# nash169/manifold-gp

Measured on AMD Instinct MI355X. Metric: CG-solve wall-time + SpMV HBM GB/s, N=60k RMNIST graph, higher is better.
Workload: dtype f32; 1 GPU; C3 RMNIST-like N=60000 d=784 k=50 nu=2 randomwalk; nodes=60000, edges=1777442, nnz_padded=3667592, rhs_columns=1, system=A = I + noise*outputscale*Q, Q=(2nu/kappa^2 I + L)^nu x D, solver=CG on A (Chronopoulos-Gear, one hipGraph per solve)

## Files before the change

include/mgp_hip.h:

```cpp
#ifndef MGP_HIP_H
#define MGP_HIP_H

#include <stddef.h>
#include <stdint.h>

#ifdef __cplusplus
extern "C" {
#endif

#define MGP_OK 0
#define MGP_ERR_ARG (-1)
#define MGP_ERR_WORKSPACE (-2)
#define MGP_ERR_UNSUPPORTED (-3)
#define MGP_ERR_NOT_CONVERGED (-4)
#define MGP_ERR_KNN_AMBIGUOUS (-5)
#define MGP_ERR_TIMEOUT (-6)

#define MGP_PAD 4

int mgp_version(void);
int mgp_device_info(int* cu_count, int* wave_size, size_t* hbm_bytes);

size_t mgp_knn_workspace_bytes(int64_t N, int64_t n, int d, int k);
int mgp_knn_search(const float* db, int64_t N, int d, const float* q, int64_t n, int k,
// ... 53 lines not shown
typedef struct {
  int64_t n;
  const int32_t* rowptr;
  const int32_t* col;
  const float* vals;
  const float* diag;
  int64_t ncols;
  const int32_t* tile_ptr;
  const int32_t* tile_cols;
  const uint16_t* lid;
  int32_t tile_rows;
  int32_t tile_max_cols;
  int32_t tile_max_entries;
  int32_t spmv_lanes;
  const int32_t* tile_rowptr;
  const float* tile_vals;
  const int32_t* tile_rowid;
  const int32_t* mt_sptr;
  const int32_t* mt_dcol;
  const float* mt_img;
  int32_t mt_tiles;
  int32_t mt_steps;
} mgp_csr_t;

int mgp_spmm_dot_blocks_csr(const mgp_csr_t* L, int C);
int mgp_spmm_set_tile_mode(int on);
int mgp_spmm_set_tile_loop_mode(int on);
int mgp_spmm_set_tile_small_mode(int on);
int mgp_spmm_set_tile_wide_mode(int on);
int mgp_spmm_set_dict_mode(int on);
int mgp_spmm_set_mt_mode(int on);
int mgp_spmm_kernel_choice(const mgp_csr_t* L, int C, int with_dot, int64_t row_offset);
int mgp_spmm_mt_fill(int64_t n, const int32_t* rowptr, const float* vals, const uint16_t* lid16, const int32_t* tile_ptr16,
                     const int32_t* tile_cols16, const int32_t* sptr, int64_t steps, int32_t* dcol, float* img, void* stream);
int mgp_spmm_timing_begin(int max_launches);
int mgp_spmm_timing_end(float* total_ms, int* launches);
int mgp_spmm_set_v4_mode(int on);

int mgp_spmm_dot_blocks(int64_t n, int C);
int mgp_spmm_set_group_hint(int lanes);
int mgp_spmm_set_rows_in_flight(int rows);
int mgp_spmm_fused(const mgp_csr_t* L, const float* X, int C, float* Y, float a, float b,
                   const float* pre, const float* post, const float* base, float cb, float co,
                   const float* dotw, float* dot_partials, void* stream);

int mgp_spmm_fused_rows(const mgp_csr_t* L_local, int64_t row_offset, const float* X, int C, float* Y,
// ... 239 lines not shown
```

manifold_gp_amd/_lib.py:

```python
import ctypes
import os
import threading
from ctypes import (POINTER, Structure, byref, c_double, c_float, c_int, c_int32, c_int64, c_size_t,
                    c_uint64, c_void_p)

import torch

_HERE = os.path.dirname(os.path.abspath(__file__))
LIB_PATH = os.path.join(_HERE, "libmgp_hip.so")
_LIB = None
_LOCK = threading.Lock()

MGP_ERRORS = {
    -1: "MGP_ERR_ARG (null pointer / bad size / bad enum)",
    -2: "MGP_ERR_WORKSPACE (work buffer too small)",
    -3: "MGP_ERR_UNSUPPORTED",
    -4: "MGP_ERR_NOT_CONVERGED",
    -5: "MGP_ERR_KNN_AMBIGUOUS",
}


class MgpError(RuntimeError):
    def __init__(self, fn, code):
        self.code = code
        what = MGP_ERRORS.get(code, "hipError_t %d" % code if code > 0 else "error %d" % code)
        super().__init__("%s failed: %s" % (fn, what))


class CsrT(Structure):
    _fields_ = [("n", c_int64), ("rowptr", c_void_p), ("col", c_void_p), ("vals", c_void_p),
                ("diag", c_void_p),
                ("ncols", c_int64), ("tile_ptr", c_void_p), ("tile_cols", c_void_p), ("lid", c_void_p),
                ("tile_rows", c_int32), ("tile_max_cols", c_int32), ("tile_max_entries", c_int32),
                ("spmv_lanes", c_int32), ("tile_rowptr", c_void_p), ("tile_vals", c_void_p),
                ("tile_rowid", c_void_p),
                ("mt_sptr", c_void_p), ("mt_dcol", c_void_p), ("mt_img", c_void_p), ("mt_tiles", c_int32), ("mt_steps", c_int32)]


class OperatorT(Structure):
    _fields_ = [("L", CsrT), ("pre", c_void_p), ("post", c_void_p), ("nu", c_int32),
                ("kappa", c_float), ("scale", c_float), ("form", c_int32), ("noise", c_float),
                ("obs_w", c_void_p)]


class CgParamsT(Structure):
    _fields_ = [("tol", c_float), ("max_iter", c_int32), ("min_iter", c_int32),
                ("stop_mode", c_int32), ("check_every", c_int32), ("use_graph", c_int32),
                ("max_refine", c_int32)]


class LanczosParamsT(Structure):
    _fields_ = [("max_basis", c_int32), ("degree", c_int32), ("max_restarts", c_int32),
                ("tol", c_float), ("seed", c_uint64)]


_P = c_void_p
SIGNATURES = {
    "mgp_version": (c_int, []),
    "mgp_device_info": (c_int, [POINTER(c_int), POINTER(c_int), POINTER(c_size_t)]),
# ... 261 lines not shown


def release_workspace(tag, device=None):
    for key in [k for k in _WORK if k[0] == tag and (device is None or k[1] == str(device))]:
        del _WORK[key]


_LEAKED = []


def leak(*objects):
    _LEAKED.extend(objects)


def csr_struct(n, rowptr, col, vals, diag, ncols=0, tiles=None, tile_vals=None, mt=None, lanes=0):
    s = CsrT(int(n), rowptr.data_ptr(), col.data_ptr(), vals.data_ptr(), diag.data_ptr(), int(ncols))
    s.spmv_lanes = int(lanes)
    if tiles is not None and (tiles.get("rowid") is None or tile_vals is not None):
        s.tile_ptr, s.tile_cols, s.lid = tiles["tile_ptr"].data_ptr(), tiles["tile_cols"].data_ptr(), tiles["lid"].data_ptr()
        s.tile_rows, s.tile_max_cols, s.tile_max_entries = tiles["rows"], tiles["max_cols"], tiles["max_entries"]
        if tiles.get("rowid") is not None:
            s.tile_rowptr, s.tile_rowid = tiles["tile_rowptr"].data_ptr(), tiles["rowid"].data_ptr()
            s.tile_vals = tile_vals.data_ptr()
    if mt is not None:
        s.mt_sptr, s.mt_dcol, s.mt_img = mt.sptr.data_ptr(), mt.dcol.data_ptr(), mt.img.data_ptr()
        s.mt_tiles, s.mt_steps = mt.tiles, mt.steps
    return s
```

manifold_gp_amd/csrc/cg.hip:

```cpp
#include <math.h>
#include <chrono>
#include <mutex>
#include <new>
#include <vector>
#include <string.h>
#include <algorithm>
#include "mgp_common.h"
#include "mgp_internal.h"
#include "cg_rule.h"
#include "cg_policy.h"
#include "cg_handoff.h"

namespace {

#ifndef MGP_LAB_UPD
#define MGP_LAB_UPD 0
#endif

typedef float mgp_cg_v4f __attribute__((ext_vector_type(4)));

struct CgArgs {
  int64_t n;
  int C, TC, TS;
  float *x, *r, *u, *w, *p, *s;
// ... 1334 lines not shown

extern "C" int mgp_cg_plan_create(const mgp_operator_t* op, int C, const float* minv,
                                  const mgp_cg_params_t* params, void* work, size_t work_bytes,
                                  void* stream, void** plan_out) {
  return plan_create_impl(op, C, minv, params, nullptr, work, work_bytes, stream, plan_out);
}

extern "C" int mgp_cg_plan_rebind(void* plan, const mgp_operator_t* op, const float* minv) {
  CgPlan* pl = static_cast<CgPlan*>(plan);
  if (!pl || !op) return MGP_ERR_ARG;
  if (pl->poisoned || pl->is_dist) return MGP_ERR_UNSUPPORTED;
  const mgp_operator_t& o = pl->op;
  const bool same = op->L.n == o.L.n && op->L.ncols == o.L.ncols && op->nu == o.nu && op->form == o.form &&
                    (op->form != 3 || ((op->obs_w != nullptr) == (o.obs_w != nullptr))) &&
                    (op->pre != nullptr) == (o.pre != nullptr) && (op->post != nullptr) == (o.post != nullptr) &&
                    (minv != nullptr) == (pl->args.minv != nullptr) &&
                    (op->L.tile_ptr != nullptr) == (o.L.tile_ptr != nullptr) && op->L.tile_rows == o.L.tile_rows &&
                    op->L.tile_max_cols == o.L.tile_max_cols && op->L.tile_max_entries == o.L.tile_max_entries &&
                    (op->L.tile_rowptr != nullptr) == (o.L.tile_rowptr != nullptr) &&
                    (op->L.tile_vals != nullptr) == (o.L.tile_vals != nullptr) &&
                    (op->L.tile_rowid != nullptr) == (o.L.tile_rowid != nullptr) &&
                    (op->L.mt_img != nullptr) == (o.L.mt_img != nullptr) && op->L.mt_tiles == o.L.mt_tiles &&
                    op->L.mt_steps == o.L.mt_steps && op->L.spmv_lanes == o.L.spmv_lanes &&
                    mgp_spmm_dot_blocks_for(&op->L, pl->C) == pl->nb_loc &&
                    (!pl->ch.fold || op->pre == op->post);
  if (!same) return MGP_ERR_UNSUPPORTED;
  if (pl->ch.cx) {
    const float cc = op->noise * op->scale;
    if (!(cc > 0.f)) return MGP_ERR_UNSUPPORTED;
    pl->opB = cx_operator(op);
    if (mgp_spmm_dot_blocks_for(&pl->opB.L, 4) != pl->cxa.nbs4) return MGP_ERR_UNSUPPORTED;
    pl->cxa.sigma = sqrtf(cc);
  }
  pl->op = mgp_operator_copy(op);
  pl->args.minv = minv;
  pl->args.pre = op->pre;
  pl->rebound = true;
  return MGP_OK;
}

extern "C" size_t mgp_cg_dist_workspace_bytes(const mgp_operator_t* op_local, int C, int world) {
  if (!op_local || C <= 0 || C > kMaxC || op_local->L.n <= 0 || world < 1 || !mgp_spmv_lanes_ok(op_local->L.spmv_lanes)) return 0;
  return cg_bytes(op_local, C, world, true);
}

extern "C" int mgp_cg_plan_create_dist(const mgp_operator_t* op_local, int C, const float* minv,
// ... 240 lines not shown
```

manifold_gp_amd/csrc/spmm.hip:

```cpp
#include <string.h>
#include <atomic>
#include <type_traits>
#include "mgp_common.h"
#include "mgp_internal.h"
#include "cg_rule.h"
#include "cg_handoff.h"
#include <hip/hip_ext.h>
#include <vector>

namespace {

constexpr int kBlock = 256;
constexpr int kMaxGrid = 4096;

struct SpmmArgs {
  int64_t n;
  const int32_t* rowptr;
  const int32_t* col;
  const float* vals;
  const float* diag;
  const float* X;
  float* Y;
  int C;
  float a, b;
// ... 189 lines not shown
  int zero;
  const unsigned grid_x = gridDim.x;
#define MGP_TILE_HEAD_ARGS                                                                                                     \
  "s"(p.n), "s"(p.rowptr), "s"(t.rowptr_t), "s"(p.vals), "s"(t.vals_t), "s"(p.diag), "s"(p.X), "s"(p.post), "s"(p.a), "s"(p.b),   \
      "s"(p.cb), "s"(p.co), "s"(t.tile_ptr), "s"(t.tile_cols), "s"(t.lid), "s"(t.max_cols), "s"(t.rowid), "s"(grid_x),           \
      "s"(PRE ? p.pre : nullptr), "s"(CBV ? p.cbv : nullptr), "s"(ONE ? (int64_t)0 : t.ntiles), "s"(ONE ? 0 : t.tiles_per_block)
  if constexpr (!STEP) {
    asm("s_mov_b32 %0, 0" : "=s"(zero) : MGP_TILE_HEAD_ARGS, "s"(p.goff), "s"(p.base), "s"(p.dotw), "s"(p.Y), "s"(p.dot_partials),
        "s"(p.copy_x), "s"(p.dot2_partials), "s"(p.skip), "s"(p.tick), "s"(p.tick_reset));
  } else {
    asm("s_mov_b32 %0, 0" : "=s"(zero) : MGP_TILE_HEAD_ARGS, "s"(cs.r), "s"(cs.x), "s"(cs.p), "s"(cs.s), "s"(cs.us), "s"(cs.pre),
        "s"(cs.pd_rr), "s"(cs.pd_delta), "s"(cs.nbs), "s"(cs.blk), "s"(cs.state), "s"(cs.host_state), "s"(cs.host_resid),
        "s"(cs.arrive), "s"(cs.tol), "s"(cs.max_iter), "s"(cs.min_iter), "s"(cs.stop_mode), "s"(cs.dcoef), "s"(cs.dgamma));
  }
#undef MGP_TILE_HEAD_ARGS
  const int32_t* __restrict__ rowptr = t.rowptr_t ? t.rowptr_t : p.rowptr;
  const float* __restrict__ vals = t.vals_t ? t.vals_t : p.vals;
  const int lane0 = __builtin_amdgcn_mbcnt_lo(0u, 0u) + zero;
  const int* __restrict__ skip_ptr = (p.skip ? p.skip : reinterpret_cast<const int*>(rowptr)) + lane0;
  const int* __restrict__ tick_ptr = (p.tick ? p.tick : reinterpret_cast<const int*>(rowptr)) + lane0;
  int skipl = 0, tickl = 0;
  constexpr int TR = BS / 4;
  constexpr int NQ = 4;
  const int lb = mgp_xcd_block(blockIdx.x, grid_x) + zero;
  const int tid = threadIdx.x, sub = tid & 3;
#ifdef MGP_STAMP
  int* st_base = !pa.stamp_on ? nullptr : (p.skip ? const_cast<int*>(p.skip) - 1 : p.tick);
  if (st_base && blockIdx.x == 0 && tid == 0) {
    const int si = atomicAdd(st_base + 8, 1);
    reinterpret_cast<unsigned long long*>(st_base + 16)[si & 255] = wall_clock64() * 8 + 0;
  }
  if (st_base && tid == 0 && blockIdx.x < 2048) reinterpret_cast<unsigned long long*>(st_base + 16)[256 + 2 * blockIdx.x] = wall_clock64();
#endif
  float* __restrict__ xl = tile_lds;
  float* __restrict__ part = tile_lds + t.max_cols;
  const float* __restrict__ x = p.X;
  const float* __restrict__ prev = p.pre;
  const int32_t* __restrict__ tile_ptr = t.tile_ptr;
  const uint32_t* __restrict__ tile_cols = reinterpret_cast<const uint32_t*>(t.tile_cols);
  const uint16_t* __restrict__ lid = t.lid;
  float dsum = 0.f, dsum2 = 0.f;
  const int64_t t0 = ONE ? (int64_t)lb : (int64_t)lb * t.tiles_per_block;
  const int64_t t1 = ONE ? t0 + 1 : (t0 + t.tiles_per_block < t.ntiles ? t0 + t.tiles_per_block : t.ntiles);
  __shared__ float cg_sh_w[MODE == kTileCgStep ? BS / MGP_WAVE : 1][3];
  __shared__ float cg_sh_o[MODE == kTileCgStep ? BS / MGP_WAVE : 1];
  __shared__ int cg_sh_state[MODE == kTileCgStep ? 2 : 1];
// ... 25 lines not shown
  };
  [[maybe_unused]] float cg_go0 = 0.f, cg_go1 = 0.f, cg_ao0 = 0.f, cg_ao1 = 0.f, cg_bb_old = 0.f;
  [[maybe_unused]] int cg_st_it = 0, cg_st_done = 0;
  [[maybe_unused]] mgp_v8i cg_blk;
  [[maybe_unused]] auto take_blk = [&]() {
    asm("" : "+s"(cg_blk));
    const CgScalars sc = __builtin_bit_cast(CgScalars, cg_blk);
    cg_go0 = sc.go0; cg_go1 = sc.go1; cg_ao0 = sc.ao0; cg_ao1 = sc.ao1; cg_bb_old = sc.bb; cg_st_it = sc.it; cg_st_done = sc.done;
  };
  [[maybe_unused]] float cg_alpha = 0.f, cg_beta = 0.f, cg_bb = 0.f, cg_nrr = 0.f;
  [[maybe_unused]] int cg_it = 0;
  [[maybe_unused]] bool cg_fresh = false;
  if constexpr (MODE == kTileCgStep) {
    static_assert(BS == 256, "the step's sums are written for four waves");
    static_assert(sizeof(CgScalars) == sizeof(mgp_v8i) && alignof(CgScalars) == alignof(mgp_v8i), "the scalar block is one load");
    cg_blk = *reinterpret_cast<const mgp_v8i*>(cs.blk);
    if constexpr (!ONE) take_blk();
    if constexpr (!CG_LATE) { cg_request_partials(); cg_sum_partials(); }
  }
  [[maybe_unused]] auto zero_x = [&]() {
    if constexpr (STEP) {
      for (int64_t tl = t0; tl < t1; ++tl) {
        const int64_t pos = tl * TR + tid;
        if (tid < TR && pos < p.n) cs.x[t.rowid ? (int64_t)t.rowid[pos] : pos] = 0.f;
      }
    }
  };
  for (int64_t tile = t0; tile < t1; ++tile) {
    if constexpr (!STEP) {
      skipl = *skip_ptr;
      tickl = *tick_ptr;
    }
    const int64_t r0 = tile * TR;
    const int64_t r1 = r0 + TR < p.n ? r0 + TR : p.n;
    const int e0 = rowptr[r0], e1 = rowptr[r1];
    const int dp = tile_ptr[tile];
    const int D = tile_ptr[tile + 1] - dp;
    const int qb = e0 >> 2, Q = (e1 - e0) >> 2;
    __builtin_amdgcn_sched_barrier(0);
    if constexpr (STEP && ONE) take_blk();
    unsigned c[NQ];
#pragma unroll
    for (int k = 0; k < NQ; ++k) {
      const int j = tid + k * BS;
      c[k] = (unsigned)tile_cols[j < D ? dp + j : 0];
    }
    __builtin_amdgcn_sched_barrier(0);
    mgp_v4f v[NQ];
    mgp_v4h l[NQ];
#pragma unroll
    for (int k = 0; k < NQ / 2; ++k) {
      const int q = tid + k * BS;
      const int qi = q < Q ? qb + q : 0;
      v[k] = *reinterpret_cast<const mgp_v4f*>(vals + 4 * (int64_t)qi);
      l[k] = *reinterpret_cast<const mgp_v4h*>(lid + 4 * (int64_t)qi);
    }
    __builtin_amdgcn_sched_barrier(0);
    float g[NQ];
#pragma unroll
    for (int k = 0; k < NQ; ++k) {
      g[k] = x[c[k]];
      if (PRE) g[k] *= prev[c[k]];
    }
    __builtin_amdgcn_sched_barrier(0);
#pragma unroll
    for (int k = NQ / 2; k < NQ; ++k) {
      const int q = tid + k * BS;
      const int qi = q < Q ? qb + q : 0;
      v[k] = *reinterpret_cast<const mgp_v4f*>(vals + 4 * (int64_t)qi);
      l[k] = *reinterpret_cast<const mgp_v4h*>(lid + 4 * (int64_t)qi);
    }
    __builtin_amdgcn_sched_barrier(0);
    const int64_t row = r0 + (tid >> 2);
    const bool valid = row < r1;
    const int64_t pr = valid ? row : r0;
    const int64_t rr = t.rowid ? (int64_t)t.rowid[pr] : pr;
    const int64_t grr = rr + p.goff;
    const int rs = rowptr[pr], re = rowptr[pr + 1];
    const float raw_x = x[grr];
    float e_x = raw_x;
    if (PRE) e_x *= prev[grr];
    const float e_diag = p.diag[rr];
    const float l_post = (p.post ? p.post : x)[grr], l_base = (p.base ? p.base : x)[grr], l_dotw = (p.dotw ? p.dotw : x)[grr];
    const float e_post = p.post ? l_post : 1.f;
    const float e_base = p.base ? l_base : 0.f;
    const float e_dotw = p.dotw ? l_dotw : 0.f;
    const float e_cb = CBV ? p.cbv[grr] : p.cb;
    [[maybe_unused]] float f_r = 0.f, f_s = 0.f, f_p = 0.f, f_x = 0.f, f_pre = 1.f;
    if constexpr (MODE == kTileCgStep) {
      f_r = cs.r[grr]; f_s = cs.s[grr]; f_p = cs.p[grr]; f_x = cs.x[grr];
      const float l_pre = (cs.us ? cs.pre : x)[grr];
      f_pre = cs.us ? l_pre : 1.f;
    }
    __builtin_amdgcn_sched_barrier(0);
    if (p.skip && skipl) return;
    if constexpr (MODE == kTileCgStep) {
      if (tile == t0) {
        if constexpr (CG_LATE) cg_request_partials();
        __builtin_amdgcn_sched_barrier(0);
// ... 1144 lines not shown
    return MGP_ERR_ARG;
  hipStream_t st = mgp_stream(stream);
  MGP_HIP_TRY(hipMemsetAsync(img, 0, (size_t)(steps + 32) * 256, st));
  MGP_HIP_TRY(hipMemsetAsync(dcol + 4 * steps, 0, 192 * sizeof(int32_t), st));
  hipLaunchKernelGGL(spmm_mt_fill_kernel, dim3((unsigned)mgp_cdiv(n + 15, kBlock)), dim3(kBlock), 0, st, n, rowptr, vals, lid16,
                     tile_ptr16, tile_cols16, sptr, dcol, img);
  MGP_LAUNCH_CHECK();
  return MGP_OK;
}


static int spmm_cols_group(int C) {
  int g = 4;
  while (g < C && g < 64) g <<= 1;
  return g;
}

static int spmm_rows_per_pass(int C, int lanes, int rows_in_flight) {
  if (C == 1) return (kBlock / lanes) * rows_in_flight;
  if (C <= 16 && (C & 3) == 0) return (kBlock / 16) * 4;
  return kBlock / spmm_cols_group(C) * 4;
}

static size_t tile_lds_bytes(const mgp_csr_t* L) {
  return ((size_t)L->tile_max_cols + (size_t)(L->tile_max_entries >> 2)) * sizeof(float);
}

static int tile_grid(const mgp_csr_t* L, int* tiles_per_block) {
  const int64_t ntiles = mgp_cdiv(L->n, L->tile_rows);
  const int64_t tpb = mgp_cdiv(ntiles, kMaxGrid);
  if (tiles_per_block) *tiles_per_block = (int)tpb;
  return (int)mgp_cdiv(ntiles, tpb);
}

static int tile_small_window(const mgp_csr_t* L) {
  const int max_q = L->tile_max_entries >> 2;
  const long budget = 40448 - (long)L->tile_max_cols * 16;
  long w = budget > 0 ? budget / 16 / 256 * 256 : 0;
  if (w < 1024) w = 1024;
  if (w > max_q) w = (max_q + 255) / 256 * 256;
  return (int)(w > 0 ? w : 256);
}
static size_t tile_small_lds_bytes(const mgp_csr_t* L, int C) {
  const size_t max_q = (size_t)(L->tile_max_entries >> 2), w = (size_t)tile_small_window(L);
  size_t b = ((size_t)L->tile_max_cols + (max_q < w ? max_q : w)) * 16;
  const size_t red = (size_t)64 * C * sizeof(float);
  return b > red ? b : red;
}

static int tile_wide_cap(const mgp_csr_t* L) {
  int cap = (L->tile_max_cols + 63) / 64 * 64;
// ... 19 lines not shown
  if (s > need) s = need;
  return (int)s;
}
static size_t dict_lds_bytes(const mgp_csr_t* L, int C) {
  const size_t d = (size_t)(dict_slots(L, C) + 1) * dict_nv(C) * 256 + (size_t)dict_stream_cap(L) * 6;
  const size_t red = (size_t)64 * dict_nv(C) * 256;
  return d > red ? d : red;
}
static int dict_grid(const mgp_csr_t* L) {
  const int64_t ntiles = mgp_cdiv(L->n, L->tile_rows);
  return (int)(ntiles < kMaxGrid ? ntiles : kMaxGrid);
}

constexpr int kMtMinCols = 48;
static bool mt_image_fits(const mgp_csr_t* L, int C) {
  if (!L->mt_img || !L->mt_sptr || !L->mt_dcol || L->mt_tiles <= 0 || L->mt_steps <= 0) return false;
  if (C < kMtMinCols || C > 256 || (C & 3) != 0 || L->tile_rowid) return false;
  if (L->ncols != 0 && L->ncols != L->n) return false;
  if ((int64_t)L->n * C * 4 >= (int64_t(1) << 31) || ((int64_t)L->mt_steps + 32) * 256 >= (int64_t(1) << 31)) return false;
  if ((L->mt_steps & 15) != 0) return false;
  return L->mt_tiles == (int32_t)mgp_cdiv(L->n, 16);
}

static TileArgs tile_args(const mgp_csr_t* L, int tiles_per_block, int part_window) {
  return TileArgs{L->tile_ptr, L->tile_cols, L->lid, mgp_cdiv(L->n, L->tile_rows), tiles_per_block, L->tile_max_cols,
                  L->tile_rowptr, L->tile_vals, L->tile_rowid, L->tile_max_entries, part_window};
}

namespace {
enum class SpmmFamily { RowGroups, Gather, TileC1, TileSmall, MatrixCore, Dict, TileWide };

struct SpmmPlan {
  int err;
  SpmmFamily family;
  int grid;
  size_t lds;
  int dot_blocks;
  bool align16;
  int64_t rows_per_block;
  int lanes, rows_in_flight;
  bool v4_ok;
  int tiles_per_block;
  bool one_tile;
  int window;
  int slots, stream_cap;
  int wide_cap;
};
}

static SpmmPlan spmm_plan(const mgp_csr_t* L, int C, int64_t row_offset, bool with_dot) {
  SpmmPlan pl{};
  pl.tiles_per_block = 1;
  if (!mgp_spmv_lanes_ok(L->spmv_lanes)) { pl.err = MGP_ERR_ARG; return pl; }
  const int tile = g_tile_mode, tile_small = g_tile_small_mode, tile_wide = g_tile_wide_mode, v4 = g_spmm_v4_mode,
            dict = g_dict_mode, mt = g_mt_mode;
  const int ord = (L->tile_rowptr != nullptr) + (L->tile_vals != nullptr) + (L->tile_rowid != nullptr);
  const bool dicts = tile && (ord == 0 || ord == 3) && L->lid && L->tile_ptr && L->tile_cols;
  const bool dicts64 = dicts && L->tile_rows == 64 && (L->tile_max_entries & 3) == 0;
  const bool wide = C > 16 && C <= 256 && (C & 3) == 0;
  const bool big_x = (size_t)L->n * (size_t)C * sizeof(float) >= ((size_t)96 << 20);

  if (C == 1 && dicts && (L->tile_rows == 32 || L->tile_rows == 64 || L->tile_rows == 128) && tile_lds_bytes(L) <= 65536 - 64) {
    pl.family = SpmmFamily::TileC1;
    pl.grid = pl.dot_blocks = tile_grid(L, &pl.tiles_per_block);
    pl.one_tile = pl.tiles_per_block == 1 && !g_tile_loop_mode;
    pl.lds = tile_lds_bytes(L);
    return pl;
  }
  if ((C == 4 || C == 8 || C == 12 || C == 16) && tile_small && dicts64 && tile_small_lds_bytes(L, C) <= 65536 - 64) {
    pl.family = SpmmFamily::TileSmall;
    pl.align16 = true;
    pl.grid = pl.dot_blocks = tile_grid(L, &pl.tiles_per_block);
    pl.lds = tile_small_lds_bytes(L, C);
    pl.window = tile_small_window(L);
    return pl;
  }
  if (mt && mt_image_fits(L, C)) {
    if (row_offset == 0) {
      pl.family = SpmmFamily::MatrixCore;
      pl.align16 = true;
      pl.grid = pl.dot_blocks = (int)mgp_cdiv((int64_t)L->mt_tiles * ((C + 63) / 64), kBlock / 64);
      return pl;
    }
    if (with_dot) { pl.err = MGP_ERR_UNSUPPORTED; return pl; }
  }
  if (wide && dict && dicts64 && dict_slots(L, C) >= 32 && (dict == 2 || (C >= 64 && big_x))) {
    pl.family = SpmmFamily::Dict;
    pl.align16 = true;
    pl.grid = pl.dot_blocks = dict_grid(L);
// ... 113 lines not shown
template <int V> using IntC = std::integral_constant<int, V>;
template <class F> static void with_pre(bool pre, F&& f) { if (pre) f(std::true_type{}); else f(std::false_type{}); }
template <class F> static void with_quads(int C, F&& f) {
  if (C == 4) f(IntC<1>{});
  else if (C == 8) f(IntC<2>{});
  else if (C == 12) f(IntC<3>{});
  else f(IntC<4>{});
}

static bool aligned16(const void* a, const void* b, const void* c = nullptr, const void* d = nullptr) {
  return ((reinterpret_cast<uintptr_t>(a) | reinterpret_cast<uintptr_t>(b) | reinterpret_cast<uintptr_t>(c) |
           reinterpret_cast<uintptr_t>(d)) & 15) == 0;
}

template <bool CB>
int spmm_launch(const SpmmPlan& pl, const mgp_csr_t* L, void* record_to, SpmmArgs& p, hipStream_t st, bool self_dot = false) {
  const int C = p.C, grid = pl.grid;
  const size_t lds = pl.lds;
  const bool pre = p.pre != nullptr;
  if (pl.align16 && !aligned16(p.X, p.Y, p.base, p.dotw)) return MGP_ERR_ARG;
  p.rows_per_block = pl.rows_per_block;
  switch (pl.family) {
  case SpmmFamily::TileC1: {
    TileArgs ta = tile_args(L, pl.tiles_per_block, 0);
    if (record_to) {
      TileLaunchRecord rec{p, ta};
      memcpy(record_to, &rec, sizeof(rec));
    }
    auto tiles = [&](auto bs, auto one) { with_pre(pre, [&](auto P) {
      constexpr int BS = decltype(bs)::value;
      constexpr bool ONE = decltype(one)::value;
      const auto kernel = self_dot ? &spmv_tile_kernel<decltype(P)::value, BS, CB, true, ONE> : &spmv_tile_kernel<decltype(P)::value, BS, CB, false, ONE>;
      if (g_spmv_timer.on && 2 * g_spmv_timer.used + 1 < (int)g_spmv_timer.ev.size()) {
        hipEvent_t e0 = g_spmv_timer.ev[2 * g_spmv_timer.used], e1 = g_spmv_timer.ev[2 * g_spmv_timer.used + 1];
        ++g_spmv_timer.used;
        hipExtLaunchKernelGGL(kernel, dim3(grid), dim3(BS), lds, st, e0, e1, 0, p, ta);
      } else hipLaunchKernelGGL(kernel, dim3(grid), dim3(BS), lds, st, p, ta);
    }); };
    auto forms = [&](auto bs) { if (pl.one_tile) tiles(bs, std::true_type{}); else tiles(bs, std::false_type{}); };
    if (L->tile_rows == 32) forms(IntC<128>{});
    else if (L->tile_rows == 64) forms(IntC<256>{});
    else forms(IntC<512>{});
  } break;
  case SpmmFamily::TileSmall: {
    TileArgs ta = tile_args(L, pl.tiles_per_block, pl.window);
    with_quads(C, [&](auto c4) { with_pre(pre, [&](auto P) {
      hipLaunchKernelGGL((spmm_tile_q_kernel<decltype(c4)::value, decltype(P)::value, CB>), dim3(grid), dim3(256), lds, st, p, ta);
// ... 104 lines not shown
#endif
  if (o.first) {
    if (pl.family != SpmmFamily::TileC1) return MGP_ERR_UNSUPPORTED;
    p.copy_x = o.first->copy_x;
    p.dot2_partials = ((dotw || self_dot) && dot_partials) ? o.first->dot2_partials : nullptr;
    p.tick_reset = o.first->tick_reset;
  }
  void* record_to = o.first ? o.first->record : nullptr;
  hipStream_t st = mgp_stream(stream);
  return o.cbv ? spmm_launch<true>(pl, L, record_to, p, st) : spmm_launch<false>(pl, L, record_to, p, st, self_dot);
}

int mgp_spmm_cgstep(const mgp_csr_t* L, const float* T, float a, float b, const float* post, float co, const MgpCgStep& cs,
                    bool decide, void* stream) {
  if (!L || !L->rowptr || !L->col || !L->vals || !L->diag || !T || L->n <= 0) return MGP_ERR_ARG;
  if (!cs.r || !cs.x || !cs.p || !cs.s || !cs.pd_rr || !cs.pd_delta || !cs.blk || !cs.state || !cs.host_state || !cs.host_resid ||
      !cs.arrive || (cs.us && !cs.pre) || T == cs.r || T == cs.us) return MGP_ERR_ARG;
  const SpmmPlan pl = spmm_plan(L, 1, 0, true);
  if (pl.err != MGP_OK) return pl.err;
  if (pl.family != SpmmFamily::TileC1 || L->tile_rows != 64 || pl.lds + kCgStepStaticLds > 65536) return MGP_ERR_UNSUPPORTED;
  if (cs.nbs != pl.dot_blocks || cs.nbs < 1 || cs.nbs > 16 * 256) return MGP_ERR_ARG;
  SpmmArgs p{L->n, L->rowptr, L->col, L->vals, L->diag, T, nullptr, 1, a, b, nullptr, post, nullptr, 1.f, co,
             nullptr, nullptr, 0, nullptr, nullptr, 0, nullptr, nullptr, 0, nullptr};
  const TileArgs ta = tile_args(L, pl.tiles_per_block, 0);
  const dim3 grid(pl.grid), block(256);
  hipStream_t st = mgp_stream(stream);
  auto step = [&](auto ds, auto one) {
    constexpr int DS = decltype(ds)::value;
    constexpr bool ONE = decltype(one)::value;
    if (decide) hipLaunchKernelGGL((spmv_tile_cgstep_kernel<256, DS, true, ONE>), grid, block, pl.lds, st, p, ta, cs);
    else hipLaunchKernelGGL((spmv_tile_cgstep_kernel<256, DS, false, ONE>), grid, block, pl.lds, st, p, ta, cs);
  };
  if (cs.nbs <= 4 * 256) { if (pl.one_tile) step(IntC<4>{}, std::true_type{}); else step(IntC<4>{}, std::false_type{}); }
  else { if (pl.one_tile) step(IntC<16>{}, std::true_type{}); else step(IntC<16>{}, std::false_type{}); }
  MGP_LAUNCH_CHECK();
  return MGP_OK;
}

extern "C" int mgp_spmm_fused(const mgp_csr_t* L, const float* X, int C, float* Y, float a, float b,
                              const float* pre, const float* post, const float* base, float cb,
                              float co, const float* dotw, float* dot_partials, void* stream) {
  return mgp_spmm_fused_opts(L, X, C, Y, a, b, pre, post, base, cb, co, dotw, dot_partials, MgpSpmmOpts{}, stream);
}

__global__ void scale_rows_kernel(const float* __restrict__ s, const float* __restrict__ x,
                                  float* __restrict__ y, int64_t n, int C) {
  int64_t total = n * C;
// ... 90 lines not shown
```

manifold_gp_amd/graph.py:

```python
import ctypes

import torch

from . import _lib
from ._lib import check, lib, ptr, stream


TILE_ROWS = 64


REORDER_BELOW_REUSE = 3.0


def bfs_order(n, rowptr, col):
    order = torch.empty(n, dtype=torch.int32, device=col.device)
    wb = lib().mgp_graph_bfs_workspace_bytes(n)
    work = _lib.workspace(wb, "graph", col.device)
    check(lib().mgp_graph_bfs_order(n, ptr(rowptr), ptr(col), ptr(order), ptr(work), work.numel(), stream()),
          "mgp_graph_bfs_order")
    return order


def chain_order(n, rowptr, col, d2):
    order = torch.empty(n, dtype=torch.int32, device=col.device)
# ... 11 lines not shown
        tile_cols = torch.empty(nnz, dtype=torch.int32, device=dev)
        lid = torch.empty(nnz, dtype=torch.int16, device=dev)
        tile_rowptr = torch.empty(n + 1, dtype=torch.int32, device=dev) if order is not None else None
        emap = torch.empty(nnz, dtype=torch.int32, device=dev) if order is not None else None
        wb = lib().mgp_graph_tiles_workspace_bytes(n, nnz)
        work = _lib.workspace(wb, "graph", dev)
        total, mc, me = ctypes.c_int64(0), ctypes.c_int32(0), ctypes.c_int32(0)
        rc = lib().mgp_graph_tiles(n, ptr(rowptr), ptr(col), nnz, rows, ptr(order), ptr(tile_rowptr), ptr(emap),
                                   ptr(tile_ptr), ptr(tile_cols), ptr(lid), ctypes.byref(total), ctypes.byref(mc),
                                   ctypes.byref(me), ptr(work), work.numel(), stream())
        if rc == -3:
            continue
        check(rc, "mgp_graph_tiles")
        if (mc.value + me.value // 4) * 4 > 65536 - 64:
            continue
        t = dict(tile_ptr=tile_ptr, tile_cols=tile_cols[:total.value].clone(), lid=lid, rows=rows,
                 max_cols=mc.value, max_entries=me.value, total_cols=total.value, reuse=nnz / max(total.value, 1))
        if order is not None:
            t.update(tile_rowptr=tile_rowptr, emap=emap.long(), rowid=order)
        return t
    return None


def require_no_self_edges(graph, stage):
    count = int(getattr(graph, "self_edges", 0))
    if count:
        raise ValueError("%s is not defined on a graph with self edges: %d coincident node%s (a repeated point whose k-NN list "
                         "does not start with itself, or an edge (i, i) of the caller's list); remove the repeated points first"
                         % (stage, count, "" if count == 1 else "s"))


WIDE_CHAIN = [True]
WIDE_CHAIN_MIN_NODES = 4096
WIDE_CHAIN_MAX_NODES = 400000
WIDE_CHAIN_GAIN = 1.25
MT_MIN_NODES = 4096
MT_MIN_FILL = 0.125
MT_ENABLED = [True]


class MtPlan:

    def __init__(self, sptr, dcol, img, tiles, steps, fill):
        self.sptr, self.dcol, self.img, self.tiles, self.steps, self.fill = sptr, dcol, img, tiles, steps, fill

    @staticmethod
# ... 19 lines not shown
        if st is None:
            return None
        t, steps = st["tiles"], st["steps"]
        dcol = torch.empty(4 * steps + 192, dtype=torch.int32, device=vals.device)
        img = torch.empty(64 * (steps + 32), dtype=torch.float32, device=vals.device)
        check(lib().mgp_spmm_mt_fill(graph.n, ptr(graph.rowptr), ptr(vals), ptr(t["lid"]), ptr(t["tile_ptr"]), ptr(t["tile_cols"]),
                                     ptr(st["sptr"]), steps, ptr(dcol), ptr(img), stream()), "mgp_spmm_mt_fill")
        return cls(st["sptr"], dcol, img, st["ntiles"], steps, st["fill"])


def morton_order(x):
    n, d = x.shape
    order = torch.empty(n, dtype=torch.int32, device=x.device)
    wb = lib().mgp_morton_order_workspace_bytes(n)
    work = _lib.workspace(wb, "graph", x.device)
    check(lib().mgp_morton_order(ptr(_lib.f32c(x)), n, d, ptr(order), ptr(work), work.numel(), stream()),
          "mgp_morton_order")
    return order


def build_tiles_auto(n, rowptr, col, nnz, points=None):
    t = build_tiles(n, rowptr, col, nnz)
    if t is None or t["reuse"] >= REORDER_BELOW_REUSE or n < 4 * TILE_ROWS:
        return t
    if points is not None and points.dim() == 2 and points.shape[1] <= 3 and points.shape[0] == n:
        order = morton_order(points)
    else:
        order = bfs_order(n, rowptr, col)
    t2 = build_tiles(n, rowptr, col, nnz, order=order)
    return t2 if (t2 is not None and t2["reuse"] > 1.3 * t["reuse"]) else t


class KnnGraph:
    _next_uid = [1]

    def __init__(self, n, tri_row, tri_col, tri_val, rowptr, col, d2, eid, tiles="auto", points=None):
        self.uid = KnnGraph._next_uid[0]
        KnnGraph._next_uid[0] += 1
        self.n = int(n)
        self.tri_row, self.tri_col, self.tri_val = tri_row, tri_col, tri_val
        self.rowptr, self.col, self.d2, self.eid = rowptr, col, d2, eid
        self.M = int(tri_val.shape[0])
        self.nnz = int(col.shape[0])
        self.self_edges = int((tri_row == tri_col).sum()) if self.M else 0
        self._edge_index = None
        if isinstance(tiles, str):
            tiles = build_tiles_auto(self.n, rowptr, col, self.nnz, points) if col.is_cuda else None
        self.tiles = tiles
        mean_row = self.nnz / max(self.n, 1)
        lanes = 8
        while lanes < 64 and lanes * 16 < mean_row:
            lanes *= 2
        self.spmv_lanes = lanes
# ... 283 lines not shown
```

manifold_gp_amd/parallel.py:

```python
import ctypes
import json
import os
import sys
import time

import torch

from . import _lib
from ._lib import CgParamsT, OperatorT, check, lib, ptr, stream


class RowPartition:

    def __init__(self, n, world, align=64):
        if n <= 0 or world <= 0:
            raise ValueError("n and world must be positive")
        self.n, self.world = int(n), int(world)
        n_loc = -(-self.n // self.world)
        self.n_loc = -(-n_loc // align) * align
        self.n_pad = self.n_loc * self.world

    def range(self, rank):
        r0 = rank * self.n_loc
        return r0, r0 + self.n_loc
# ... 149 lines not shown
        newest = ref & ~inc
        out.append(torch.nonzero(newest, as_tuple=False).squeeze(-1))
        inc |= newest
    return out


class PartitionedOperator:

    def __init__(self, desc, part, rank):
        from .graph import build_tiles
        if desc.form not in (0, 2):
            raise ValueError("the partitioned solver takes single-chain operators (forms 0 and 2)")
        d = desc.data
        g = d.graph
        if g.n != part.n_pad:
            raise ValueError("the operator must live on the padded graph (pad_graph): %d != %d" % (g.n, part.n_pad))
        self.desc, self.part, self.rank = desc, part, rank
        r0, r1 = part.range(rank)
        nu = int(desc.nu)
        if part.world == 1:
            self.tiles, self.vals_t = g.tiles, d.vals_t
            if self.tiles is None:
                raise RuntimeError("the partitioned solver needs the tile view of the graph")
            self.launch_rows = [g.n] * nu
            self.ghosts = [torch.empty(0, dtype=torch.int64, device=g.device) for _ in range(nu - 1)]
        else:
            self.ghosts = ghost_layers(g, r0, r1, nu - 1)
            inc = torch.zeros(g.n, dtype=torch.bool, device=g.device)
            inc[r0:r1] = True
            for gl in self.ghosts:
                inc[gl] = True
            rest = torch.nonzero(~inc, as_tuple=False).squeeze(-1)
            order = torch.cat([torch.arange(r0, r1, device=g.device)] + self.ghosts + [rest]).to(torch.int32)
            self.tiles = build_tiles(g.n, g.rowptr, g.col, g.nnz, order=order)
            if self.tiles is None:
                raise RuntimeError("no tile view for this row order (a tile exceeds the LDS budget)")
            self.vals_t = d.vals.index_select(0, self.tiles["emap"])
            tr = self.tiles["rows"]
            sizes = [part.n_loc]
            for gl in self.ghosts:
                sizes.append(sizes[-1] + int(gl.numel()))
            self.launch_rows = [min(g.n, -(-sizes[nu - 1 - s] // tr) * tr) for s in range(nu)]
        self.op = desc.struct()
        self.op.L = _lib.csr_struct(g.n, g.rowptr, g.col, d.vals, d.diag, tiles=self.tiles, tile_vals=self.vals_t,
                                    lanes=g.spmv_lanes)
        self.ghost_rows = sum(int(gl.numel()) for gl in self.ghosts)
# ... 386 lines not shown
```

Baseline: 3960 GB/s (algorithmic SpMV bytes inside the CG solve).

## Add nnz-balanced tile cut for single-column tiled SpMV

Adds an alternative tiling for the C=1 tiled SpMV path that cuts rows into tiles capped at a fixed number of nonzeros, instead of fixed 64-row tiles. Each tile is padded to 64 rows and a per-tile shift maps padded rows back to real rows. The metadata is passed through the existing tile_rowptr slot, tagged with a magic number. The aim is to even out per-workgroup work and LDS use on skewed-degree graphs, at the cost of more tiles, extra padded-row bookkeeping and a host-side preprocessing pass.

```diff
diff --git a/include/mgp_hip.h b/include/mgp_hip.h
--- a/include/mgp_hip.h
+++ b/include/mgp_hip.h
@@ -99,6 +99,23 @@
   int32_t mt_tiles;
   int32_t mt_steps;
 } mgp_csr_t;
+
+typedef struct {
+  int64_t magic;
+  int64_t n;
+  const int32_t* tile_ptr;
+  const int32_t* tile_cols;
+  const uint16_t* lid;
+  const int32_t* rowptr_pad;
+  const int32_t* tile_shift;
+  int32_t tiles;
+  int32_t max_cols;
+  int32_t max_entries;
+  int32_t reserved;
+} mgp_c1_tiles_t;
+#define MGP_C1_TILES_MAGIC 0x31435f5053474d4dLL
+
+#define MGP_C1_TILE_CAP 4096
 
 int mgp_spmm_dot_blocks_csr(const mgp_csr_t* L, int C);
 int mgp_spmm_set_tile_mode(int on);
diff --git a/manifold_gp_amd/_lib.py b/manifold_gp_amd/_lib.py
--- a/manifold_gp_amd/_lib.py
+++ b/manifold_gp_amd/_lib.py
@@ -35,6 +35,18 @@
                 ("spmv_lanes", c_int32), ("tile_rowptr", c_void_p), ("tile_vals", c_void_p),
                 ("tile_rowid", c_void_p),
                 ("mt_sptr", c_void_p), ("mt_dcol", c_void_p), ("mt_img", c_void_p), ("mt_tiles", c_int32), ("mt_steps", c_int32)]
+
+
+class C1TilesT(Structure):
+    _fields_ = [("magic", c_int64), ("n", c_int64), ("tile_ptr", c_void_p), ("tile_cols", c_void_p), ("lid", c_void_p),
+                ("rowptr_pad", c_void_p), ("tile_shift", c_void_p), ("tiles", c_int32), ("max_cols", c_int32),
+                ("max_entries", c_int32), ("reserved", c_int32)]
+
+
+C1_TILES_MAGIC = 0x31435f5053474d4d
+
+
+C1_BALANCED = [True]
 
 
 class OperatorT(Structure):
@@ -342,6 +354,9 @@
         if tiles.get("rowid") is not None:
             s.tile_rowptr, s.tile_rowid = tiles["tile_rowptr"].data_ptr(), tiles["rowid"].data_ptr()
             s.tile_vals = tile_vals.data_ptr()
+        c1 = tiles.get("c1") if C1_BALANCED[0] else None
+        if c1 is not None and tiles.get("rowid") is None and not ncols and c1["struct"].n == int(n):
+            s.tile_rowptr = ctypes.addressof(c1["struct"])
     if mt is not None:
         s.mt_sptr, s.mt_dcol, s.mt_img = mt.sptr.data_ptr(), mt.dcol.data_ptr(), mt.img.data_ptr()
         s.mt_tiles, s.mt_steps = mt.tiles, mt.steps
diff --git a/manifold_gp_amd/csrc/cg.hip b/manifold_gp_amd/csrc/cg.hip
--- a/manifold_gp_amd/csrc/cg.hip
+++ b/manifold_gp_amd/csrc/cg.hip
@@ -1380,6 +1380,7 @@
                     (op->L.tile_rowid != nullptr) == (o.L.tile_rowid != nullptr) &&
                     (op->L.mt_img != nullptr) == (o.L.mt_img != nullptr) && op->L.mt_tiles == o.L.mt_tiles &&
                     op->L.mt_steps == o.L.mt_steps && op->L.spmv_lanes == o.L.spmv_lanes &&
+                    (op->L.tile_vals || op->L.tile_rowid || op->L.tile_rowptr == o.L.tile_rowptr) &&
                     mgp_spmm_dot_blocks_for(&op->L, pl->C) == pl->nb_loc &&
                     (!pl->ch.fold || op->pre == op->post);
   if (!same) return MGP_ERR_UNSUPPORTED;
diff --git a/manifold_gp_amd/csrc/spmm.hip b/manifold_gp_amd/csrc/spmm.hip
--- a/manifold_gp_amd/csrc/spmm.hip
+++ b/manifold_gp_amd/csrc/spmm.hip
@@ -235,6 +235,9 @@
   int skipl = 0, tickl = 0;
   constexpr int TR = BS / 4;
   constexpr int NQ = 4;
+  static_assert(BS != 256 || 4 * NQ * BS == MGP_C1_TILE_CAP, "the balanced cut caps a tile at what a 256-lane workgroup holds in registers");
+  const int shm = -(((t.rowptr_t != nullptr && t.rowid == nullptr) ? 1 : 0) + lane0);
+  int sh0 = 0, shd = 0;
   const int lb = mgp_xcd_block(blockIdx.x, grid_x) + zero;
   const int tid = threadIdx.x, sub = tid & 3;
 #ifdef MGP_STAMP
@@ -306,7 +309,7 @@
     if constexpr (STEP) {
       for (int64_t tl = t0; tl < t1; ++tl) {
         const int64_t pos = tl * TR + tid;
-        if (tid < TR && pos < p.n) cs.x[t.rowid ? (int64_t)t.rowid[pos] : pos] = 0.f;
+        if (tid < TR - shd && pos < p.n) cs.x[t.rowid ? (int64_t)t.rowid[pos] : pos - sh0] = 0.f;
       }
     }
   };
@@ -328,6 +331,11 @@
     for (int k = 0; k < NQ; ++k) {
       const int j = tid + k * BS;
       c[k] = (unsigned)tile_cols[j < D ? dp + j : 0];
+      if (k == 0) {
+        const int64_t si = ((TR * (int)grid_x + 1) & shm) + (int)tile;
+        sh0 = rowptr[si];
+        shd = rowptr[si + 1];
+      }
     }
     __builtin_amdgcn_sched_barrier(0);
     mgp_v4f v[NQ];
@@ -355,10 +363,12 @@
       l[k] = *reinterpret_cast<const mgp_v4h*>(lid + 4 * (int64_t)qi);
     }
     __builtin_amdgcn_sched_barrier(0);
+    shd = (shd - sh0) & shm;
+    sh0 &= shm;
     const int64_t row = r0 + (tid >> 2);
-    const bool valid = row < r1;
+    const bool valid = row < r1 - shd;
     const int64_t pr = valid ? row : r0;
-    const int64_t rr = t.rowid ? (int64_t)t.rowid[pr] : pr;
+    const int64_t rr = t.rowid ? (int64_t)t.rowid[pr] : pr - sh0;
     const int64_t grr = rr + p.goff;
     const int rs = rowptr[pr], re = rowptr[pr + 1];
     const float raw_x = x[grr];
@@ -1549,11 +1559,34 @@
   return kBlock / spmm_cols_group(C) * 4;
 }
 
-static size_t tile_lds_bytes(const mgp_csr_t* L) {
+static const mgp_c1_tiles_t* c1_set(const mgp_csr_t* L) {
+  if (!L->tile_rowptr || L->tile_vals || L->tile_rowid) return nullptr;
+  const mgp_c1_tiles_t* s = reinterpret_cast<const mgp_c1_tiles_t*>(L->tile_rowptr);
+  return s->magic == MGP_C1_TILES_MAGIC ? s : nullptr;
+}
+static const int32_t* order_rowptr(const mgp_csr_t* L) { return (L->tile_vals || L->tile_rowid) ? L->tile_rowptr : nullptr; }
+
+static bool c1_balanced(const mgp_csr_t* L, int C, int64_t row_offset) {
+  if (C != 1 || row_offset != 0) return false;
+  const mgp_c1_tiles_t* s = c1_set(L);
+  if (!s || !s->tile_ptr || !s->tile_cols || !s->lid || !s->rowptr_pad || !s->tile_shift) return false;
+  if (L->tile_rows != 64 || s->n != L->n) return false;
+  if (L->ncols != 0 && L->ncols != L->n) return false;
+  if (s->tiles < 1 || s->tiles > kMaxGrid || (s->max_entries & 3) != 0) return false;
+  if (s->tile_shift != s->rowptr_pad + ((int64_t)s->tiles * 64 + 1)) return false;
+  return (int64_t)s->tiles * 64 >= L->n && L->n >= s->tiles;
+}
+
+static size_t tile_lds_bytes(const mgp_csr_t* L, bool balanced = false) {
+  if (balanced) return ((size_t)c1_set(L)->max_cols + (size_t)(c1_set(L)->max_entries >> 2)) * sizeof(float);
   return ((size_t)L->tile_max_cols + (size_t)(L->tile_max_entries >> 2)) * sizeof(float);
 }
 
-static int tile_grid(const mgp_csr_t* L, int* tiles_per_block) {
+static int tile_grid(const mgp_csr_t* L, int* tiles_per_block, bool balanced = false) {
+  if (balanced) {
+    if (tiles_per_block) *tiles_per_block = 1;
+    return c1_set(L)->tiles;
+  }
   const int64_t ntiles = mgp_cdiv(L->n, L->tile_rows);
   const int64_t tpb = mgp_cdiv(ntiles, kMaxGrid);
   if (tiles_per_block) *tiles_per_block = (int)tpb;
@@ -1619,9 +1652,14 @@
   return L->mt_tiles == (int32_t)mgp_cdiv(L->n, 16);
 }
 
-static TileArgs tile_args(const mgp_csr_t* L, int tiles_per_block, int part_window) {
+static TileArgs tile_args(const mgp_csr_t* L, int tiles_per_block, int part_window, bool balanced = false) {
+  if (balanced) {
+    const mgp_c1_tiles_t* s = c1_set(L);
+    return TileArgs{s->tile_ptr, s->tile_cols, s->lid, s->tiles, 1, s->max_cols, s->rowptr_pad, nullptr, nullptr,
+                    s->max_entries, part_window};
+  }
   return TileArgs{L->tile_ptr, L->tile_cols, L->lid, mgp_cdiv(L->n, L->tile_rows), tiles_per_block, L->tile_max_cols,
-                  L->tile_rowptr, L->tile_vals, L->tile_rowid, L->tile_max_entries, part_window};
+                  order_rowptr(L), L->tile_vals, L->tile_rowid, L->tile_max_entries, part_window};
 }
 
 namespace {
@@ -1639,6 +1677,7 @@
   bool v4_ok;
   int tiles_per_block;
   bool one_tile;
+  bool balanced;
   int window;
   int slots, stream_cap;
   int wide_cap;
@@ -1651,7 +1690,7 @@
   if (!mgp_spmv_lanes_ok(L->spmv_lanes)) { pl.err = MGP_ERR_ARG; return pl; }
   const int tile = g_tile_mode, tile_small = g_tile_small_mode, tile_wide = g_tile_wide_mode, v4 = g_spmm_v4_mode,
             dict = g_dict_mode, mt = g_mt_mode;
-  const int ord = (L->tile_rowptr != nullptr) + (L->tile_vals != nullptr) + (L->tile_rowid != nullptr);
+  const int ord = (order_rowptr(L) != nullptr) + (L->tile_vals != nullptr) + (L->tile_rowid != nullptr);
   const bool dicts = tile && (ord == 0 || ord == 3) && L->lid && L->tile_ptr && L->tile_cols;
   const bool dicts64 = dicts && L->tile_rows == 64 && (L->tile_max_entries & 3) == 0;
   const bool wide = C > 16 && C <= 256 && (C & 3) == 0;
@@ -1659,9 +1698,10 @@
 
   if (C == 1 && dicts && (L->tile_rows == 32 || L->tile_rows == 64 || L->tile_rows == 128) && tile_lds_bytes(L) <= 65536 - 64) {
     pl.family = SpmmFamily::TileC1;
-    pl.grid = pl.dot_blocks = tile_grid(L, &pl.tiles_per_block);
+    pl.balanced = c1_balanced(L, C, row_offset) && tile_lds_bytes(L, true) <= 65536 - 64;
+    pl.grid = pl.dot_blocks = tile_grid(L, &pl.tiles_per_block, pl.balanced);
     pl.one_tile = pl.tiles_per_block == 1 && !g_tile_loop_mode;
-    pl.lds = tile_lds_bytes(L);
+    pl.lds = tile_lds_bytes(L, pl.balanced);
     return pl;
   }
   if ((C == 4 || C == 8 || C == 12 || C == 16) && tile_small && dicts64 && tile_small_lds_bytes(L, C) <= 65536 - 64) {
@@ -1821,7 +1861,8 @@
   p.rows_per_block = pl.rows_per_block;
   switch (pl.family) {
   case SpmmFamily::TileC1: {
-    TileArgs ta = tile_args(L, pl.tiles_per_block, 0);
+    TileArgs ta = tile_args(L, pl.tiles_per_block, 0, pl.balanced);
+    if (pl.balanced) p.n = (int64_t)c1_set(L)->tiles * 64;
     if (record_to) {
       TileLaunchRecord rec{p, ta};
       memcpy(record_to, &rec, sizeof(rec));
@@ -1972,7 +2013,8 @@
   if (cs.nbs != pl.dot_blocks || cs.nbs < 1 || cs.nbs > 16 * 256) return MGP_ERR_ARG;
   SpmmArgs p{L->n, L->rowptr, L->col, L->vals, L->diag, T, nullptr, 1, a, b, nullptr, post, nullptr, 1.f, co,
              nullptr, nullptr, 0, nullptr, nullptr, 0, nullptr, nullptr, 0, nullptr};
-  const TileArgs ta = tile_args(L, pl.tiles_per_block, 0);
+  const TileArgs ta = tile_args(L, pl.tiles_per_block, 0, pl.balanced);
+  if (pl.balanced) p.n = (int64_t)c1_set(L)->tiles * 64;
   const dim3 grid(pl.grid), block(256);
   hipStream_t st = mgp_stream(stream);
   auto step = [&](auto ds, auto one) {
diff --git a/manifold_gp_amd/graph.py b/manifold_gp_amd/graph.py
--- a/manifold_gp_amd/graph.py
+++ b/manifold_gp_amd/graph.py
@@ -57,6 +57,83 @@
     return None
 
 
+C1_TILE_CAP = 4096
+C1_MAX_TILES = 4096
+C1_FOLD_PARTIALS = 1024
+C1_BALANCED = _lib.C1_BALANCED
+
+
+def c1_balanced_cut(rowptr, rows=TILE_ROWS, cap=C1_TILE_CAP):
+    rp = torch.as_tensor(rowptr, dtype=torch.int64, device="cpu").contiguous()
+    n = int(rp.numel()) - 1
+    first, r = [0], 0
+    while r < n:
+        e = int(torch.searchsorted(rp, rp[r] + cap, right=True)) - 1
+        e = max(min(e, r + rows, n), r + 1)
+        first.append(e)
+        r = e
+    return torch.tensor(first, dtype=torch.int64)
+
+
+def c1_padded_positions(rowptr, first, rows=TILE_ROWS):
+    rp = torch.as_tensor(rowptr, dtype=torch.int64, device="cpu")
+    T = int(first.numel()) - 1
+    pos = torch.arange(rows * T + 1, dtype=torch.int64)
+    t = torch.clamp(pos // rows, max=max(T - 1, 0))
+    row = torch.minimum(first[t] + (pos - rows * t), first[t + 1]) if T else torch.zeros(1, dtype=torch.int64)
+    return rp[row], rows * torch.arange(T + 1, dtype=torch.int64) - first
+
+
+def c1_balanced_policy(rowptr, rows=TILE_ROWS, ordered=False):
+    if ordered or rows != 64:
+        return None
+    rp = torch.as_tensor(rowptr, dtype=torch.int64, device="cpu")
+    n = int(rp.numel()) - 1
+    fixed = -(-n // rows)
+    if n < 1 or fixed > C1_MAX_TILES:
+        return None
+    edges = rp[torch.clamp(torch.arange(fixed + 1, dtype=torch.int64) * rows, max=n)]
+    if int((edges[1:] - edges[:-1]).max()) <= C1_TILE_CAP:
+        return None
+    first = c1_balanced_cut(rp, rows)
+    T = int(first.numel()) - 1
+    if T > C1_MAX_TILES or (fixed <= C1_FOLD_PARTIALS < T):
+        return None
+    return first
+
+
+def c1_balanced_tiles(n, rowptr, col, nnz, tiles):
+    if tiles is None or nnz <= 0 or not col.is_cuda:
+        return None
+    first = c1_balanced_policy(rowptr.cpu(), tiles["rows"], ordered=tiles.get("rowid") is not None)
+    if first is None:
+        return None
+    dev = col.device
+    T = int(first.numel()) - 1
+    rp_pad, shift = c1_padded_positions(rowptr.cpu(), first)
+    both = torch.cat([rp_pad, shift]).to(torch.int32).to(dev)
+    rowptr_pad, shift = both[:64 * T + 1], both[64 * T + 1:]
+    tile_ptr = torch.empty(T + 1, dtype=torch.int32, device=dev)
+    tile_cols = torch.empty(nnz, dtype=torch.int32, device=dev)
+    lid = torch.empty(nnz, dtype=torch.int16, device=dev)
+    work = _lib.workspace(lib().mgp_graph_tiles_workspace_bytes(64 * T, nnz), "graph", dev)
+    total, mc, me = ctypes.c_int64(0), ctypes.c_int32(0), ctypes.c_int32(0)
+    rc = lib().mgp_graph_tiles(64 * T, ptr(rowptr_pad), ptr(col), nnz, 64, None, None, None, ptr(tile_ptr), ptr(tile_cols),
+                               ptr(lid), ctypes.byref(total), ctypes.byref(mc), ctypes.byref(me), ptr(work), work.numel(),
+                               stream())
+    if rc == -3:
+        return None
+    check(rc, "mgp_graph_tiles")
+    if (mc.value + me.value // 4) * 4 > 65536 - 64 or (me.value & 3):
+        return None
+    tile_cols = tile_cols[:total.value].clone()
+    desc = _lib.C1TilesT(_lib.C1_TILES_MAGIC, int(n), tile_ptr.data_ptr(), tile_cols.data_ptr(), lid.data_ptr(), rowptr_pad.data_ptr(),
+                         shift.data_ptr(), T, mc.value, me.value, 0)
+    return dict(tile_ptr=tile_ptr, tile_cols=tile_cols, lid=lid, rowptr_pad=rowptr_pad, struct=desc,
+                tile_shift=shift, T=T, max_cols=mc.value, max_entries=me.value,
+                total_cols=total.value, first=first)
+
+
 def require_no_self_edges(graph, stage):
     count = int(getattr(graph, "self_edges", 0))
     if count:
@@ -122,13 +199,21 @@
 def build_tiles_auto(n, rowptr, col, nnz, points=None):
     t = build_tiles(n, rowptr, col, nnz)
     if t is None or t["reuse"] >= REORDER_BELOW_REUSE or n < 4 * TILE_ROWS:
-        return t
+        return with_c1_balanced(t, n, rowptr, col, nnz)
     if points is not None and points.dim() == 2 and points.shape[1] <= 3 and points.shape[0] == n:
         order = morton_order(points)
     else:
         order = bfs_order(n, rowptr, col)
     t2 = build_tiles(n, rowptr, col, nnz, order=order)
-    return t2 if (t2 is not None and t2["reuse"] > 1.3 * t["reuse"]) else t
+    return t2 if (t2 is not None and t2["reuse"] > 1.3 * t["reuse"]) else with_c1_balanced(t, n, rowptr, col, nnz)
+
+
+def with_c1_balanced(t, n, rowptr, col, nnz):
+    if t is not None and t.get("rowid") is None:
+        c1 = c1_balanced_tiles(n, rowptr, col, nnz, t)
+        if c1 is not None:
+            t["c1"] = c1
+    return t
 
 
 class KnnGraph:
diff --git a/manifold_gp_amd/parallel.py b/manifold_gp_amd/parallel.py
--- a/manifold_gp_amd/parallel.py
+++ b/manifold_gp_amd/parallel.py
@@ -195,6 +195,7 @@
             self.tiles, self.vals_t = g.tiles, d.vals_t
             if self.tiles is None:
                 raise RuntimeError("the partitioned solver needs the tile view of the graph")
+            self.tiles = {k: v for k, v in self.tiles.items() if k != "c1"}
             self.launch_rows = [g.n] * nu
             self.ghosts = [torch.empty(0, dtype=torch.int64, device=g.device) for _ in range(nu - 1)]
         else:
```

Measured after the change: 4109 GB/s (algorithmic SpMV bytes inside the CG solve), median of 6. 1.04x the previous value.
